# torchmd/mdgrad

Measured on AMD Instinct MI355X. Metric: MD steps/sec (fwd+adjoint), 108-atom LJ NHC, higher is better.
Workload: dtype f32; 1 GPU; FCC 3^3 LJ(1,1) 108 atoms rc 2.5 NHC(Q50,5) dt 0.005, 49 steps+RDF loss+adjoint, 16384 rep/GPU; replicas_per_gpu=16384, md_steps_per_pass=802816, parallelism=replica-dp1, rdf_fused_into_trajectory_kernels=True

## Files before the change

mdgrad_amd/csrc/traj_ring.hpp:

```cpp

__device__ __forceinline__ float ring_move(float v, int src4) {
    return __builtin_bit_cast(float, __builtin_amdgcn_ds_bpermute(src4, __builtin_bit_cast(int, v)));
}
__device__ __forceinline__ f32x2 ring_move(f32x2 v, int src4) { return f32x2{ring_move(v.x, src4), ring_move(v.y, src4)}; }
__device__ __forceinline__ float row_up(float v) {
    return __builtin_bit_cast(float, __builtin_amdgcn_update_dpp(0, __builtin_bit_cast(int, v), 0x101, 0xf, 0xf, true));
}
__device__ __forceinline__ float row_down(float v) {
    return __builtin_bit_cast(float, __builtin_amdgcn_update_dpp(0, __builtin_bit_cast(int, v), 0x111, 0xf, 0xf, true));
}
__device__ __forceinline__ float lane0(float v) {
    return __builtin_bit_cast(float, __builtin_amdgcn_readfirstlane(__builtin_bit_cast(int, v)));
}
__device__ __forceinline__ f32x2 rcp2(f32x2 v) { return f32x2{__builtin_amdgcn_rcpf(v.x), __builtin_amdgcn_rcpf(v.y)}; }
__device__ __forceinline__ float hsum(f32x2 v) { return v.x + v.y; }

__device__ __forceinline__ f32x2 min_image_diag2_near_fused(f32x2 d, float invf, float h) {
    const float M = 12582912.f;
    const f32x2 o = __builtin_elementwise_fma(d, f32x2{invf, invf}, f32x2{M, M}) - M;
    return d - o * h;
}

struct Vec3x2 { f32x2 x, y, z; };
__device__ __forceinline__ Vec3x2 vzero() { const f32x2 z = {0.f, 0.f}; return Vec3x2{z, z, z}; }
__device__ __forceinline__ Vec3x2 ring_move(const Vec3x2& a, int s) { return Vec3x2{ring_move(a.x, s), ring_move(a.y, s), ring_move(a.z, s)}; }

struct RingLJ {
    float sig2, rc2, m1a, m1b, ka, kb, tsa, tsb, tea, teb;
    float a6, a12, b6, b12, sg6, sg12;
    float ivx, ivy, ivz, hx, hy, hz;
    float fvx, fvy, fvz;
    TermConst t0;
    uint32_t rcm;
    bool full;
};

__device__ __forceinline__ RingLJ ring_constants(const TrajArgs& A, int m = 0) {
    const TermConst t0 = term_prepare(A.terms.t[m], A.theta);
    const float e4 = 4.f * t0.k1, cq = t0.c;
    RingLJ K;
    K.sig2 = t0.k0 * t0.k0; K.rc2 = t0.rc2;
    K.m1a = 6.f * e4 * cq; K.m1b = 12.f * e4;
    K.ka = (42.f + 6.f) * e4 * cq; K.kb = (156.f + 12.f) * e4;
    K.tsa = 18.f * e4 * t0.k2 * cq; K.tsb = 72.f * e4 * t0.k2;
    K.tea = 12.f * cq; K.teb = 24.f;
    K.sg6 = K.sig2 * K.sig2 * K.sig2; K.sg12 = K.sg6 * K.sg6;
    K.a6 = K.m1a * K.sg6; K.a12 = K.m1b * K.sg12; K.b6 = K.ka * K.sg6; K.b12 = K.kb * K.sg12;
    K.ivx = A.cell.inv[0]; K.ivy = A.cell.inv[4]; K.ivz = A.cell.inv[8];
    K.hx = A.cell.h[0]; K.hy = A.cell.h[4]; K.hz = A.cell.h[8];
    K.t0 = t0;
    K.rcm = t0.rc2 > 0.f ? __float_as_uint(t0.rc2) - 1u : 0u;
    K.fvx = A.inv_f[0]; K.fvy = A.inv_f[1]; K.fvz = A.inv_f[2];
    K.full = A.lean && A.fused_image && !(A.prm.n_atoms & 1);
    return K;
}

struct RingRdf {
    uint32_t* hist; float inv_h, tlo, fmax;
    const float4* tab; float ulo, inv_hu, tmax;
    float toff, tzero;
    const float2* ttab; unsigned long long* tg64; int32_t* tflag; float tgw, tu0, tinv_du, ttmax, tlim; int tgmax;
};

__device__ __forceinline__ void ring_table_scatter2(const RingRdf& X, int idx, float va, float vb) {
    if (!(fmaxf(fabsf(va), fabsf(vb)) < X.tlim)) *X.tflag = 4;
    atomicAdd(X.tg64 + idx, fx64(va));
    atomicAdd(X.tg64 + idx + 1, fx64(vb));
}

constexpr bool ring_level_force(int level) { return level == 1 || level == 2; }

template <int LEVEL, int IMAGE, bool CROSS, bool JSIDE, int RDF, int KIND, bool SUMS = true>
__device__ __forceinline__ void ring_pair(const RingLJ& K, const RingRdf& X, const Vec3x2& qi, const Vec3x2& wi,
                                          const Vec3x2& qj, const Vec3x2& wj, bool v0, bool v1, bool r0, bool r1,
                                          Vec3x2& fi, Vec3x2& gi, Vec3x2& fj, Vec3x2& gj, f32x2 (&TH)[MDG_MAX_THETA],
                                          Vec3x2& ri, Vec3x2& rj) {
    f32x2 dx = (CROSS ? qj.x.yx : qj.x) - qi.x, dy = (CROSS ? qj.y.yx : qj.y) - qi.y,
          dz = (CROSS ? qj.z.yx : qj.z) - qi.z;
// ... 165 lines not shown
    const bool vi0 = 2 * lane < N, vi1 = 2 * lane + 1 < N;
    f32x2* sqx = lds; f32x2* sqy = lds + 64; f32x2* sqz = lds + 128;
    f32x2* swx = lds + 192; f32x2* swy = lds + 256; f32x2* swz = lds + 320;
    ring_lds_fence();
    sqx[lane] = q.x; sqy[lane] = q.y; sqz[lane] = q.z;
    if constexpr (LEVEL >= 2) { swx[lane] = w.x; swy[lane] = w.y; swz[lane] = w.z; }
    ring_lds_fence();
    Vec3x2 fi = vzero(), gi = vzero(), fj = vzero(), gj = vzero(), ri = vzero(), rj = vzero();
    f32x2 S[MDG_MAX_THETA], D[MDG_MAX_THETA];
#pragma unroll
    for (int k = 0; k < MDG_MAX_THETA; ++k) { S[k] = f32x2{0.f, 0.f}; D[k] = S[k]; }
    static_assert(!FULL || !MASK, "the full ring has no selection mask");
    static_assert(!FULL || NEAR, "the full ring runs on the window form of the minimum image");
    constexpr int IMAGE = NEAR ? (FULL ? 2 : 1) : 0;
    const int nsteps = (nl - 1) >> 1;
    if (!FULL || lane < nl) {
    {
        const bool v = FULL || (vi0 && vi1);
        bool vm = v;
        if constexpr (MASK) vm = v && ((ring_mask_word(M.w, lane >> 4) >> (2 * (lane & 15) + 1)) & 1u);
        ring_pair<LEVEL, IMAGE, true, false, RDF, KIND, SUMS>(K, X, q, w, q, w, vm, vm, v, RDF == 2 && v, fi, gi, fj, gj, D, ri, rj);
    }
    const int prev = lane < nl ? ((lane == 0 ? nl : lane) - 1) * 4 : lane * 4;
    int idx = lane;
    Vec3x2 qj, wj = vzero();
#pragma unroll 1
    for (int k = 1; k <= nsteps; ++k) {
        idx -= 1; idx = idx < 0 ? idx + nl : idx;
        qj.x = sqx[idx]; qj.y = sqy[idx]; qj.z = sqz[idx];
        if constexpr (ring_level_force(LEVEL)) fj = ring_move(fj, prev);
        if constexpr (LEVEL >= 2) { wj.x = swx[idx]; wj.y = swy[idx]; wj.z = swz[idx]; gj = ring_move(gj, prev); }
        if constexpr (RDF == 2) rj = ring_move(rj, prev);
        const bool vj0 = FULL || 2 * idx < N, vj1 = FULL || 2 * idx + 1 < N;
        const bool s0 = FULL || (vi0 && vj0), s1 = FULL || (vi1 && vj1), c0 = FULL || (vi0 && vj1), c1 = FULL || (vi1 && vj0);
        bool ms0 = s0, ms1 = s1, mc0 = c0, mc1 = c1;
        if constexpr (MASK) {
            const uint32_t b0 = ring_mask_word(M.w, idx >> 4) >> (2 * (idx & 15)), b1 = ring_mask_word(M.w + 4, idx >> 4) >> (2 * (idx & 15));
            ms0 = s0 && (b0 & 1u); mc0 = c0 && (b0 & 2u); mc1 = c1 && (b1 & 1u); ms1 = s1 && (b1 & 2u);
        }
        ring_pair<LEVEL, IMAGE, false, true, RDF, KIND, SUMS>(K, X, q, w, qj, wj, ms0, ms1, s0, s1, fi, gi, fj, gj, S, ri, rj);
        ring_pair<LEVEL, IMAGE, true, true, RDF, KIND, SUMS>(K, X, q, w, qj, wj, mc0, mc1, c0, c1, fi, gi, fj, gj, S, ri, rj);
    }
    if (!(nl & 1)) {
        idx -= 1; idx = idx < 0 ? idx + nl : idx;
        qj.x = sqx[idx]; qj.y = sqy[idx]; qj.z = sqz[idx];
        if constexpr (LEVEL >= 2) { wj.x = swx[idx]; wj.y = swy[idx]; wj.z = swz[idx]; }
        const bool vj0 = FULL || 2 * idx < N, vj1 = FULL || 2 * idx + 1 < N;
        const bool s0 = FULL || (vi0 && vj0), s1 = FULL || (vi1 && vj1), c0 = FULL || (vi0 && vj1), c1 = FULL || (vi1 && vj0);
        bool ms0 = s0, ms1 = s1, mc0 = c0, mc1 = c1;
        if constexpr (MASK) {
            const uint32_t b0 = ring_mask_word(M.w, idx >> 4) >> (2 * (idx & 15)), b1 = ring_mask_word(M.w + 4, idx >> 4) >> (2 * (idx & 15));
            ms0 = s0 && (b0 & 1u); mc0 = c0 && (b0 & 2u); mc1 = c1 && (b1 & 1u); ms1 = s1 && (b1 & 2u);
        }
        const bool once = RDF == 2 || 2 * lane < nl;
        Vec3x2 fu = vzero(), gu = vzero(), ru = vzero();
        ring_pair<LEVEL, IMAGE, false, false, RDF, KIND, SUMS>(K, X, q, w, qj, wj, ms0, ms1, s0 && once, s1 && once, fi, gi, fu, gu, D, ri, ru);
        ring_pair<LEVEL, IMAGE, true, false, RDF, KIND, SUMS>(K, X, q, w, qj, wj, mc0, mc1, c0 && once, c1 && once, fi, gi, fu, gu, D, ri, ru);
    }
    }
    int home = lane + nsteps; home = home >= nl ? home - nl : home;
    home = (lane < nl ? home : lane) * 4;
    if constexpr (ring_level_force(LEVEL)) {
        fj = ring_move(fj, home);
        f.x = fi.x + fj.x; f.y = fi.y + fj.y; f.z = fi.z + fj.z;
    }
    if constexpr (LEVEL >= 2) {
        gj = ring_move(gj, home);
        g.x = -(gi.x + gj.x); g.y = -(gi.y + gj.y); g.z = -(gi.z + gj.z);
        if constexpr (SUMS) {
#pragma unroll
            for (int k = 0; k < MDG_MAX_THETA; ++k)
                th[k] = 2.f * hsum(S[k]) + hsum(D[k]);
        }
    }
    if constexpr (RDF == 2) {
        rj = ring_move(rj, home);
        rq.x = ri.x + rj.x; rq.y = ri.y + rj.y; rq.z = ri.z + rj.z;
    } else {
        rq = vzero();
    }
}

__device__ __forceinline__ bool ring_near(const RingLJ& K, const Vec3x2& q) {
    const f32x2 sx = q.x * K.ivx, sy = q.y * K.ivy, sz = q.z * K.ivz;
    bool out = false;
    out |= !(sx.x > -0.24f && sx.x < 1.24f) | !(sx.y > -0.24f && sx.y < 1.24f);
    out |= !(sy.x > -0.24f && sy.x < 1.24f) | !(sy.y > -0.24f && sy.y < 1.24f);
    out |= !(sz.x > -0.24f && sz.x < 1.24f) | !(sz.y > -0.24f && sz.y < 1.24f);
    return __builtin_amdgcn_ballot_w64(out) == 0;
}

template <int LEVEL, int RDF, int KIND, bool MASK, bool SUMS = true>
__device__ __forceinline__ void ring_force(const RingLJ& K, const RingRdf& X, const RingMask& M, bool with_rdf, int N, int lane,
                                           const Vec3x2& q, const Vec3x2& w, Vec3x2& f, Vec3x2& g, float (&th)[MDG_MAX_THETA],
                                           Vec3x2& rq, f32x2* __restrict__ lds) {
    const bool near = ring_near(K, q);
    constexpr bool FULL_OK = !MASK && KIND == KIND_LJ126;
    const bool full = FULL_OK && near && K.full;
    if constexpr (RDF != 0) {
        if (with_rdf) {
            if (full) ring_sweep<LEVEL, true, RDF, KIND, MASK, SUMS, FULL_OK>(K, X, M, N, lane, q, w, f, g, th, rq, lds);
            else if (near) ring_sweep<LEVEL, true, RDF, KIND, MASK, SUMS>(K, X, M, N, lane, q, w, f, g, th, rq, lds);
            else ring_sweep<LEVEL, false, RDF, KIND, MASK, SUMS>(K, X, M, N, lane, q, w, f, g, th, rq, lds);
            return;
        }
    }
    if constexpr (LEVEL >= 1) {
        if (full) ring_sweep<LEVEL, true, 0, KIND, MASK, SUMS, FULL_OK>(K, X, M, N, lane, q, w, f, g, th, rq, lds);
        else if (near) ring_sweep<LEVEL, true, 0, KIND, MASK, SUMS>(K, X, M, N, lane, q, w, f, g, th, rq, lds);
        else ring_sweep<LEVEL, false, 0, KIND, MASK, SUMS>(K, X, M, N, lane, q, w, f, g, th, rq, lds);
// ... 346 lines not shown
        gth[0] += nve ? (gs * 0.5f * h) * 2.f : gs * h;
        gth[1] += nve ? (ge * 0.5f * h) * 2.f : ge * h;
    } else {
#pragma unroll
        for (int k = 0; k < kind_ntheta(KIND); ++k) {
            const float tk = wave_sum(th[k]);
            gth[k] += nve ? (tk * 0.5f * h) * 2.f : tk * h;
        }
    }
}

constexpr int RING_TABLE_WAVES = 8;
constexpr int RING_RDF_ADJ_WAVES = 4;
constexpr int ring_adj_waves(bool rdf, int kind) { return kind == KIND_TABLE ? RING_TABLE_WAVES : (rdf ? RING_RDF_ADJ_WAVES : 1); }
constexpr int RING_PARK_VECS = 4;
constexpr bool ring_adj_parks(int kind, bool mask, int nt, bool ft) { return kind == KIND_LJ126 && !mask && nt == 1 && ft; }
constexpr int ring_adj_slab(bool parks) { return (6 + (parks ? 3 * RING_PARK_VECS : 0)) * 64; }
__device__ __forceinline__ void ring_park(f32x2* __restrict__ park, int slot, int lane, const Vec3x2& a) {
    f32x2* p = park + slot * 192 + lane;
    p[0] = a.x; p[64] = a.y; p[128] = a.z;
}
__device__ __forceinline__ Vec3x2 ring_unpark(const f32x2* __restrict__ park, int slot, int lane) {
    const f32x2* p = park + slot * 192 + lane;
    return Vec3x2{p[0], p[64], p[128]};
}

template <bool NHC, bool RDF, int KIND, bool MASK, int NT, bool FT>
__device__ __forceinline__ void ring_adj_intervals(const TrajArgs& A, const RingRdfArgs& F, const RingLJ (&K)[NT], RingRdf& X,
                                                   const RingMask (&M)[NT], bool live, size_t fr, int lane, f32x2* __restrict__ lds,
                                                   Vec3x2& lv, Vec3x2& lq, float& lp, float (&gth)[NT][MDG_MAX_THETA]) {
    constexpr bool PARK = ring_adj_parks(KIND, MASK, NT, FT);
    static_assert(NT == 1 || !RDF, "several terms: no fused observable");
    const int N = A.prm.n_atoms, T = A.prm.n_frames, C = A.prm.n_chains, N3 = 3 * N;
    f32x2* park = lds + 6 * 64;
    f32x2 ms = {1.f, 1.f};
    if (2 * lane < N) ms.x = A.mass[2 * lane];
    if (2 * lane + 1 < N) ms.y = A.mass[2 * lane + 1];
    const f32x2 ims = rcp2(ms);
    const float Qk = ring_chain_mass(A, lane);
    const float iQ0 = 1.f / A.prm.Q[0];
    for (int i = T - 1; i >= 1; --i) {
        const float h = A.t[i] - A.t[i - 1];
        Vec3x2 q = ring_load(A.q_t + (fr + i) * N3, N, lane);
        float pv = (NHC && lane < C) ? A.pv_t[(fr + i) * C + lane] : 0.f;
        Vec3x2 w, f, dq, rq = vzero(), ru;
        float th[NT][MDG_MAX_THETA];
        if constexpr (NHC) { w.x = lv.x * ims; w.y = lv.y * ims; w.z = lv.z * ims; } else w = lv;
        const bool with_rdf = RDF && ring_frame_selected(F, i);
        if constexpr (KIND == KIND_TABLE) X.tgw = (NHC || !live) ? 0.f : 0.5f * h * A.terms.t[0].c;
        if constexpr (PARK) {
            if constexpr (NHC) ring_park(park, 0, lane, lv);
            ring_park(park, 1, lane, lq);
        }
        ring_force_terms<FT ? 3 : 2, RDF ? 2 : 0, KIND, MASK, NT, !NHC>(K, X, M, with_rdf, N, lane, q, w, f, dq, th, rq, lds);
        if constexpr (PARK) {
            if constexpr (NHC) lv = ring_unpark(park, 0, lane); else lv = w;
            lq = ring_unpark(park, 1, lane);
        }
        if constexpr (FT) f = ring_load(A.f_t + (fr + i) * N3, N, lane);
        Vec3x2 v = ring_load(A.v_t + (fr + i) * N3, N, lane);
        if (with_rdf) { lq.x += rq.x; lq.y += rq.y; lq.z += rq.z; }
        Vec3x2 lvh, lqh;
        if constexpr (NHC) {
            const Vec3x2 p{v.x * ms, v.y * ms, v.z * ms};
            const float ke = 0.5f * wave_sum(ring_dot(p, v)), slv = wave_sum(ring_dot(lv, v));
            const float pv0 = lane0(pv), lp0 = lane0(lp), c0 = pv0 * iQ0;
            const float pb = ring_bath_rhs(A, lane, Qk, pv, ke), gp = ring_bath_vjp(A, lane, Qk, pv, lp, slv);
            const float hh = 0.5f * h;
#define MDG_RING_HALF(c)                                                                     \
            {                                                                                \
                const f32x2 a = (f.c - c0 * p.c) * ims;                                      \
                const f32x2 Gv = -c0 * lv.c + lq.c + 2.f * ms * v.c * lp0;                   \
                const f32x2 vhalf = 0.5f * (-a) * h;                     \
                q.c = q.c + (v.c + vhalf) * h;                           \
                v.c = v.c + vhalf;                                                           \
                lvh.c = lv.c + Gv * hh;                                            \
                lqh.c = lq.c + dq.c * hh;                                          \
            }
            MDG_RING_HALF(x) MDG_RING_HALF(y) MDG_RING_HALF(z)
#undef MDG_RING_HALF
            const float lph = lp + gp * hh;
            pv = pv + 0.5f * (-pb) * h;
            w.x = lvh.x * ims; w.y = lvh.y * ims; w.z = lvh.z * ims;
            if constexpr (KIND == KIND_TABLE) X.tgw = live ? 0.5f * h * A.terms.t[0].c : 0.f;
            if constexpr (PARK) {
                ring_park(park, 0, lane, lv); ring_park(park, 1, lane, lq);
                ring_park(park, 2, lane, lvh); ring_park(park, 3, lane, lqh);
            }
            ring_force_terms<2, 0, KIND, MASK, NT>(K, X, M, false, N, lane, q, w, f, dq, th, ru, lds);
            if constexpr (PARK) {
                lv = ring_unpark(park, 0, lane); lq = ring_unpark(park, 1, lane);
                lvh = ring_unpark(park, 2, lane); lqh = ring_unpark(park, 3, lane);
            }
            const float slm = wave_sum(ring_dot(lvh, v));
            const float cm = lane0(pv) * iQ0, lpm0 = lane0(lph);
            const float gpm = ring_bath_vjp(A, lane, Qk, pv, lph, slm);
            const Vec3x2 gv = A.g_v ? ring_load(A.g_v + (fr + i - 1) * N3, N, lane) : vzero();
            const Vec3x2 gq = A.g_q ? ring_load(A.g_q + (fr + i - 1) * N3, N, lane) : vzero();
#define MDG_RING_FULL(c)                                                                     \
            {                                                                                \
                const f32x2 Gv = -cm * lvh.c + lqh.c + 2.f * ms * v.c * lpm0;                \
                lv.c = (lv.c + Gv * h) + gv.c;                               \
                lq.c = (lq.c + dq.c * h) + gq.c;                                   \
            }
            MDG_RING_FULL(x) MDG_RING_FULL(y) MDG_RING_FULL(z)
#undef MDG_RING_FULL
            float nlp = lp + gpm * h;
// ... 40 lines not shown
    constexpr int NWV = ring_adj_waves(RDF, KIND);
    const int wid = NWV > 1 ? __builtin_amdgcn_readfirstlane((int)(threadIdx.x >> 6)) : 0, lane = threadIdx.x & 63, N3 = 3 * N;
    const bool live = NWV == 1 || (int)(blockIdx.x * NWV + wid) < A.prm.n_rep;
    const int rep = NWV == 1 ? (int)blockIdx.x : (live ? (int)(blockIdx.x * NWV + wid) : A.prm.n_rep - 1);
    RingLJ K[NT];
    RingMask M[NT];
#pragma unroll
    for (int m = 0; m < NT; ++m) {
        K[m] = ring_constants(A, m);
        M[m] = RingMask{};
        if constexpr (MASK) M[m] = ring_mask_load(A.terms.t[m].mask, N, lane);
    }
    RingRdf X{};
    int ntab = 0;
    if constexpr (RDF) {
        float hu;
        int ncell;
        rdf_u_grid(F.mu, F.nbins, F.reach_bins, X.ulo, hu, ncell);
        float4* tab = reinterpret_cast<float4*>(smr);
        for (int n = threadIdx.x; n < ncell; n += blockDim.x) tab[n] = F.tab[n];
        if (threadIdx.x == 0) tab[ncell] = make_float4(0.f, 0.f, 0.f, 0.f);
        X.tab = tab; X.inv_hu = 1.0f / hu; X.toff = -X.ulo * X.inv_hu; X.tzero = (float)ncell;
        X.tmax = fminf((float)ncell, (F.rc * F.rc - X.ulo) * X.inv_hu);
        ntab = ncell + 1;
        __syncthreads();
    }
    f32x2* lds = reinterpret_cast<f32x2*>(smr + 4 * ntab) + wid * ring_adj_slab(ring_adj_parks(KIND, MASK, NT, FT));
    if constexpr (KIND == KIND_TABLE) {
        const MdgPairTerm& t0 = A.terms.t[0];
        float2* ttab = reinterpret_cast<float2*>(smr + 4 * ntab + NWV * 6 * 64 * 2);
        unsigned long long* tg = reinterpret_cast<unsigned long long*>(ttab + t0.p);
        int32_t* tflag = reinterpret_cast<int32_t*>(tg + 2 * t0.p);
        const float* thp = A.theta + t0.theta_off;
        for (int g = threadIdx.x; g < t0.p; g += blockDim.x) ttab[g] = make_float2(thp[2 * g], thp[2 * g + 1]);
        for (int g = threadIdx.x; g < 2 * t0.p; g += blockDim.x) tg[g] = 0ull;
        if (threadIdx.x == 0) *tflag = 0;
        X.ttab = ttab; X.tg64 = tg; X.tflag = tflag; X.tgw = 0.f;
        X.tlim = fx64_limit((double)NWV * (double)(T > 1 ? T - 1 : 1) * (double)N * (double)N);
        X.tu0 = t0.a; X.tinv_du = 1.f / t0.phi; X.ttmax = (float)(t0.p - 1); X.tgmax = t0.p - 2;
        __syncthreads();
    }
    const size_t fr = (size_t)rep * T;
    Vec3x2 lv = A.g_v ? ring_load(A.g_v + (fr + T - 1) * N3, N, lane) : vzero();
    Vec3x2 lq = A.g_q ? ring_load(A.g_q + (fr + T - 1) * N3, N, lane) : vzero();
    float lp = (nhc && lane < C && A.g_pv) ? A.g_pv[(fr + T - 1) * C + lane] : 0.f;
    float gth[NT][MDG_MAX_THETA];
#pragma unroll
    for (int m = 0; m < NT; ++m)
#pragma unroll
        for (int k = 0; k < MDG_MAX_THETA; ++k) gth[m][k] = 0.f;
    if (nhc) ring_adj_intervals<true, RDF, KIND, MASK, NT, FT>(A, F, K, X, M, live, fr, lane, lds, lv, lq, lp, gth);
    else ring_adj_intervals<false, RDF, KIND, MASK, NT, FT>(A, F, K, X, M, live, fr, lane, lds, lv, lq, lp, gth);
    if constexpr (RDF) {
        if (ring_frame_selected(F, 0)) {
            const Vec3x2 q = ring_load(A.q_t + fr * N3, N, lane), wu = vzero();
            Vec3x2 fu, gu, rq = vzero();
            float tu[MDG_MAX_THETA];
            ring_force<0, 2, KIND, MASK>(K[0], X, M[0], true, N, lane, q, wu, fu, gu, tu, rq, lds);
            lq.x += rq.x; lq.y += rq.y; lq.z += rq.z;
        }
    }
    if (live) {
        ring_store(A.adj_v0 + (size_t)rep * N3, lv, N, lane);
        ring_store(A.adj_q0 + (size_t)rep * N3, lq, N, lane);
        if (nhc && lane < C && A.adj_pv0) A.adj_pv0[(size_t)rep * C + lane] = lp;
    }
    if constexpr (KIND == KIND_TABLE) {
        __syncthreads();
        if (A.adj_theta) {
            const int M2 = 2 * A.terms.t[0].p, KT = A.terms.n_theta_total;
            const bool worst = (*X.tflag & 4) != 0;
            const double inv = 1.0 / (double)A.terms.t[0].c;
            float* out = A.adj_theta + (size_t)(blockIdx.x * NWV) * KT + A.terms.t[0].theta_off;
            for (int g = threadIdx.x; g < M2; g += blockDim.x)
                out[g] = worst ? __builtin_inff() : (float)((double)(long long)X.tg64[g] * inv);
            if (wid > 0 && live) {
                float* mine = A.adj_theta + (size_t)rep * KT + A.terms.t[0].theta_off;
                for (int g = lane; g < M2; g += 64) mine[g] = 0.f;
            }
        }
        return;
    }
    if (live && lane == 0 && A.adj_theta) {
#pragma unroll
        for (int m = 0; m < NT; ++m) {
            float* out = A.adj_theta + (size_t)rep * A.terms.n_theta_total + A.terms.t[m].theta_off;
#pragma unroll
            for (int k = 0; k < MDG_MAX_THETA; ++k)
                if (k < A.terms.t[m].n_theta) out[k] = gth[m][k];
        }
    }
}
```

mdgrad_amd/csrc/traj_small.hip:

```cpp
#include "common.hpp"
#include <cmath>

namespace {

struct TrajArgs {
    MdgTrajParams prm;
    MdgCell cell;
    MdgTerms terms;
    const float* theta;
    const float* mass;
    const float* t;
    const float* v0; const float* q0; const float* pv0;
    float* v_t; float* q_t; float* pv_t;
    const float* g_v; const float* g_q; const float* g_pv;
    float* adj_v0; float* adj_q0; float* adj_pv0; float* adj_theta;
    int32_t* nonfinite;
    int ld;
    uint16_t* code;
    int freq;
    long long count0;
    float* f_t;
    int lean;
    float inv_f[3];
    int fused_image;
};

constexpr int KMAX_ALL = MDG_MAX_TERMS * MDG_MAX_THETA;
constexpr int RED_FLOATS = 16 * (KMAX_ALL + 2);
#define KMAX (NT * MDG_MAX_THETA)

template <int LEVEL, int LDC, bool EVEN, bool NEAR>
__device__ __forceinline__ void force_lj126_packed(const TrajArgs& A, int tpa_log2, const float* __restrict__ q,
                                                   const float* __restrict__ w, float* __restrict__ f,
                                                   float* __restrict__ dq, float& th_sig, float& th_eps, bool th_on) {
    const int N = A.prm.n_atoms, LD = LDC ? LDC : A.ld;
    const int TPA = 1 << tpa_log2;
    const int slots = blockDim.x >> tpa_log2;
    const int slot = threadIdx.x >> tpa_log2, sub = threadIdx.x & (TPA - 1);
    const TermConst t0 = term_prepare(A.terms.t[0], A.theta);
    const float sig2 = t0.k0 * t0.k0, e4 = 4.f * t0.k1, cq = t0.c, rc2 = t0.rc2;
    const float m1a = 6.f * e4 * cq, m1b = 12.f * e4;
    const float ka = (42.f + 6.f) * e4 * cq, kb = (156.f + 12.f) * e4;
    const float tsa = 18.f * e4 * t0.k2 * cq, tsb = 72.f * e4 * t0.k2;
    const float tea = 12.f * cq, teb = 24.f;
    const float ivx = A.cell.inv[0], ivy = A.cell.inv[4], ivz = A.cell.inv[8];
    const float hx = A.cell.h[0], hy = A.cell.h[4], hz = A.cell.h[8];
    f32x2 S6 = {0.f, 0.f}, S12 = {0.f, 0.f};
    for (int i = slot; i < N; i += slots) {
        const float xi = q[i], yi = q[LD + i], zi = q[2 * LD + i];
        float wxi = 0.f, wyi = 0.f, wzi = 0.f;
        if (LEVEL >= 2) { wxi = w[i]; wyi = w[LD + i]; wzi = w[2 * LD + i]; }
        f32x2 fx = {0.f, 0.f}, fy = fx, fz = fx, gx = fx, gy = fx, gz = fx;
#pragma unroll 2
        for (int j = 2 * sub; j < N; j += 2 * TPA) {
            const bool live2 = EVEN || j + 1 < N;
            const float* qj = q + j;
            const f32x2 qx = *reinterpret_cast<const f32x2*>(qj), qy = *reinterpret_cast<const f32x2*>(qj + LD),
                        qz = *reinterpret_cast<const f32x2*>(qj + 2 * LD);
            f32x2 dx = qx - xi, dy = qy - yi, dz = qz - zi;
            f32x2 ax = {0.f, 0.f}, ay = ax, az = ax;
            if (LEVEL >= 2) {
                const float* wj = w + j;
                ax = wxi - *reinterpret_cast<const f32x2*>(wj); ay = wyi - *reinterpret_cast<const f32x2*>(wj + LD);
                az = wzi - *reinterpret_cast<const f32x2*>(wj + 2 * LD);
            }
            if constexpr (NEAR) {
                dx = min_image_diag2_near(dx, ivx, hx); dy = min_image_diag2_near(dy, ivy, hy);
                dz = min_image_diag2_near(dz, ivz, hz);
            } else {
                dx = min_image_diag2(dx, ivx, hx); dy = min_image_diag2(dy, ivy, hy); dz = min_image_diag2(dz, ivz, hz);
            }
            const f32x2 d2 = norm2_ref2(dx, dy, dz);
            const bool ok0 = (d2.x != 0.f) && (d2.x < rc2);
            const bool ok1 = live2 && (d2.y != 0.f) && (d2.y < rc2);
            const f32x2 i2 = {ok0 ? __builtin_amdgcn_rcpf(d2.x) : 0.f, ok1 ? __builtin_amdgcn_rcpf(d2.y) : 0.f};
            const f32x2 s2 = sig2 * i2;
            const f32x2 s6 = s2 * s2 * s2;
// ... 671 lines not shown
        }
        return;
    }
    if (tid == 0 && A.adj_theta) {
        const int KT = A.terms.n_theta_total;
#pragma unroll
        for (int m = 0; m < NT; ++m)
#pragma unroll
            for (int k = 0; k < MDG_MAX_THETA; ++k)
                if (m < A.terms.n_terms && k < A.terms.t[m].n_theta)
                    A.adj_theta[(size_t)rep * KT + A.terms.t[m].theta_off + k] = gth[m * MDG_MAX_THETA + k];
    }
}

#include "traj_ring.hpp"

constexpr int RING_TABLE_MAX_NODES = 2048;
size_t ring_table_adj_lds(int nodes);
size_t device_lds_per_block() {
    static size_t cached = 0;
    if (!cached) {
        int dev = 0, v = 0;
        if (hipGetDevice(&dev) != hipSuccess || hipDeviceGetAttribute(&v, hipDeviceAttributeMaxSharedMemoryPerBlock, dev) != hipSuccess || v <= 0)
            v = 64 * 1024;
        cached = (size_t)v;
    }
    return cached;
}

int ring_kind(const MdgPairTerm& t);
bool ring_form(const MdgTrajParams& p, const MdgCell& cell, const MdgTerms& terms) {
    const MdgPairTerm& t = terms.t[0];
    if (t.kind == MDG_PAIR_TABLE) {
        const char* e = getenv("MDG_RING_TABLE");
        return !(e && e[0] == '0') && terms.n_terms == 1 && cell.diag && !t.mask && t.p <= RING_TABLE_MAX_NODES && p.n_atoms <= 128 &&
               ring_table_adj_lds(t.p) <= device_lds_per_block();
    }
    if (terms.n_terms == 2 || terms.n_terms == 3) {
        bool any_mask = false;
        for (int m = 0; m < terms.n_terms; ++m) {
            const MdgPairTerm& u = terms.t[m];
            if (u.kind != MDG_PAIR_LJ || ring_kind(u) != ring_kind(t)) return false;
            any_mask = any_mask || u.mask != nullptr;
        }
        return cell.diag && p.n_atoms <= 128 && any_mask;
    }
    return terms.n_terms == 1 && cell.diag && (!t.mask || t.kind == MDG_PAIR_LJ) && t.kind >= 0 && t.kind <= MDG_PAIR_YUKAWA &&
           p.n_atoms <= 128;
}
int ring_lean() {
    static const int lean = [] { const char* e = getenv("MDG_RING_LEAN"); return !(e && e[0] == '0') ? 1 : 0; }();
    return lean;
}
bool fused_image_multiplier(float h, float inv, float* out) {
    if (!(h > 0.f) || !(inv > 0.f) || !std::isfinite(h) || !std::isfinite(inv)) return false;
    auto rounded = [inv](float d) { volatile float s = d * inv; return (float)s; };
    float tau = 0.5f * h;
    if (!(tau > 0.f) || !std::isfinite(rounded(2.f * h))) return false;
    int budget = 64;
    while (rounded(std::nextafterf(tau, 0.f)) > 0.5f && --budget > 0) tau = std::nextafterf(tau, 0.f);
    while (!(rounded(tau) > 0.5f) && --budget > 0) tau = std::nextafterf(tau, INFINITY);
    if (budget <= 0) return false;
    const double below = (double)std::nextafterf(tau, 0.f), at = (double)tau;
    for (int k = 0; k <= 8; ++k) {
        float c = inv;
        const int steps = (k + 1) / 2;
        for (int s = 0; s < steps; ++s) c = std::nextafterf(c, (k & 1) ? 0.f : INFINITY);
        if (below * (double)c <= 0.5 && 0.5 < at * (double)c) { *out = c; return true; }
    }
    return false;
}
void set_fused_image(TrajArgs& a) {
    a.fused_image = a.cell.diag ? 1 : 0;
    for (int k = 0; k < 3; ++k) {
        a.inv_f[k] = a.cell.inv[4 * k];
        if (a.fused_image && !fused_image_multiplier(a.cell.h[4 * k], a.cell.inv[4 * k], &a.inv_f[k])) a.fused_image = 0;
    }
}
bool use_ring(const MdgTrajParams& p, const MdgCell& cell, const MdgTerms& terms) {
    return ring_form(p, cell, terms) && (p.block == 64 || (p.block == 0 && p.n_rep >= 1024));
}
int ring_kind(const MdgPairTerm& t) {
    if (t.kind == MDG_PAIR_TABLE) return KIND_TABLE;
    return (t.kind == MDG_PAIR_LJ && t.p == 12 && (t.q == 6 || t.c == 0.f)) ? KIND_LJ126 : t.kind;
}
size_t ring_table_lds(const MdgTerms& terms, bool adjoint) {
    if (terms.t[0].kind != MDG_PAIR_TABLE) return 0;
    return sizeof(float) * (size_t)(adjoint ? 6 : 2) * terms.t[0].p + 16;
}
#define MDG_RING_FT , true
#define MDG_RING_LAUNCH(KERNEL, RDF_, TAIL, grid, block, lds, st, ...)                                        \
    do {                                                                                                      \
        const bool masked_ = terms->t[0].mask != nullptr;                                                     \
        const int nt_ = terms->n_terms;               \
        switch (ring_kind(terms->t[0])) {                                                                     \
        case KIND_LJ126:                                                                                      \
            if (nt_ == 2) hipLaunchKernelGGL((KERNEL<false, KIND_LJ126, true, 2 TAIL>), grid, block, lds, st, __VA_ARGS__);    \
            else if (nt_ == 3) hipLaunchKernelGGL((KERNEL<false, KIND_LJ126, true, 3 TAIL>), grid, block, lds, st, __VA_ARGS__); \
            else if (masked_) hipLaunchKernelGGL((KERNEL<RDF_, KIND_LJ126, true, 1 TAIL>), grid, block, lds, st, __VA_ARGS__);    \
            else hipLaunchKernelGGL((KERNEL<RDF_, KIND_LJ126, false, 1 TAIL>), grid, block, lds, st, __VA_ARGS__);               \
            break;                                                                                            \
        case MDG_PAIR_LJ:                                                                                     \
            if (nt_ == 2) hipLaunchKernelGGL((KERNEL<false, MDG_PAIR_LJ, true, 2 TAIL>), grid, block, lds, st, __VA_ARGS__);   \
            else if (nt_ == 3) hipLaunchKernelGGL((KERNEL<false, MDG_PAIR_LJ, true, 3 TAIL>), grid, block, lds, st, __VA_ARGS__);  \
            else if (masked_) hipLaunchKernelGGL((KERNEL<RDF_, MDG_PAIR_LJ, true, 1 TAIL>), grid, block, lds, st, __VA_ARGS__);   \
            else hipLaunchKernelGGL((KERNEL<RDF_, MDG_PAIR_LJ, false, 1 TAIL>), grid, block, lds, st, __VA_ARGS__);              \
// ... 162 lines not shown
    const char* who = small_who(false, o);
    const bool stale = o.extra == SmallOpt::STALE, rdf = o.extra == SmallOpt::RDF;
    MDG_CHECK_ARG(mass && t_grid && v0 && q0 && v_t && q_t && (!rdf || ((theta || terms->n_theta_total == 0) && o.raw)),
                  "%s: null buffer", who);
    MDG_CHECK_ARG(prm->ensemble == 1 || (pv0 && pv_t), "%s: NHC needs pv0/pv_t", who);
    RdfFinePlan P;
    if ((rc = validate_small_opt(who, prm, cell, terms, o, &P)) != MDG_OK) return rc;
    TrajArgs a{};
    a.prm = *prm; a.cell = *cell; a.terms = *terms; a.theta = theta; a.mass = mass; a.t = t_grid;
    a.v0 = v0; a.q0 = q0; a.pv0 = pv0; a.v_t = v_t; a.q_t = q_t; a.pv_t = pv_t; a.nonfinite = nonfinite;
    hipStream_t st = (hipStream_t)stream;
    if (rdf || (!stale && use_ring(*prm, *cell, *terms))) {
        MDG_CHECK_ARG(theta || terms->n_theta_total == 0, "%s: null theta", who);
        a.f_t = o.f_t; a.lean = ring_lean(); set_fused_image(a);
        if (!rdf) {
            MDG_RING_LAUNCH(traj_fwd_ring_kernel, false, , dim3(prm->n_rep), dim3(64), RING_LDS_FWD + ring_table_lds(*terms, false),
                            st, a, RingRdfArgs{});
            MDG_CHECK_LAUNCH("traj_fwd_ring_kernel");
            return MDG_OK;
        }
        uint32_t* ghist = nullptr;
        MDG_HIP(hipMallocAsync((void**)&ghist, sizeof(uint32_t) * (size_t)P.nfine, st));
        MDG_HIP(hipMemsetAsync(ghist, 0, sizeof(uint32_t) * (size_t)P.nfine, st));
        RingRdfArgs F = ring_rdf_args(*o.rdf, P);
        F.ghist = ghist;
        int grid = (prm->n_rep + RING_RDF_WAVES - 1) / RING_RDF_WAVES;
        if (grid > 256) grid = 256;
        const size_t lds = sizeof(float) * (size_t)((P.nfine + 1) & ~1LL) + RING_RDF_WAVES * RING_LDS_FWD;
        MDG_RING_LAUNCH(traj_fwd_ring_kernel, true, , dim3(grid), dim3(64 * RING_RDF_WAVES), lds, st, a, F);
        rc = mdg_rdf_fine_finish(ghist, P, o.rdf->mu, o.rdf->nbins, o.raw, st);
        (void)hipFreeAsync(ghist, st);
        if (rc) return rc;
        MDG_CHECK_LAUNCH("traj_fwd_ring_kernel<rdf>");
        return MDG_OK;
    }
    SmallGeom g;
    if ((rc = small_geometry(who, prm, terms, theta, false, &g)) != MDG_OK) return rc;
    a.ld = g.ld;
    if (stale) { a.code = o.code; a.freq = o.freq; a.count0 = o.count0; }
    MDG_TRAJ_DISPATCH(traj_fwd_kernel, stale);
    MDG_CHECK_LAUNCH(stale ? "traj_fwd_kernel (stale lists)" : "traj_fwd_kernel");
    return MDG_OK;
}

int traj_adj_small_run(const MdgTrajParams* prm, const MdgCell* cell, const MdgTerms* terms,
                       const float* theta, const float* mass, const float* t_grid,
                       const float* v_t, const float* q_t, const float* pv_t,
                       const float* g_v, const float* g_q, const float* g_pv,
                       float* adj_v0, float* adj_q0, float* adj_pv0, float* adj_theta, void* stream, const SmallOpt& o) {
    int rc = validate(prm, cell, terms);
    if (rc) return rc;
    const char* who = small_who(true, o);
    const bool stale = o.extra == SmallOpt::STALE, rdf = o.extra == SmallOpt::RDF;
    MDG_CHECK_ARG(mass && t_grid && v_t && q_t && adj_v0 && adj_q0 &&
                  (!rdf || ((theta || terms->n_theta_total == 0) && o.g_raw)), "%s: null buffer", who);
    MDG_CHECK_ARG(prm->ensemble == 1 || pv_t, "%s: NHC needs pv_t", who);
    RdfFinePlan P;
    if ((rc = validate_small_opt(who, prm, cell, terms, o, &P)) != MDG_OK) return rc;
    TrajArgs a{};
    a.prm = *prm; a.cell = *cell; a.terms = *terms; a.theta = theta; a.mass = mass; a.t = t_grid;
    a.v_t = const_cast<float*>(v_t); a.q_t = const_cast<float*>(q_t); a.pv_t = const_cast<float*>(pv_t);
    a.g_v = g_v; a.g_q = g_q; a.g_pv = g_pv;
    a.adj_v0 = adj_v0; a.adj_q0 = adj_q0; a.adj_pv0 = adj_pv0; a.adj_theta = adj_theta;
    hipStream_t st = (hipStream_t)stream;
    if (rdf || (!stale && use_ring(*prm, *cell, *terms))) {
        MDG_CHECK_ARG(theta || terms->n_theta_total == 0, "%s: null theta", who);
        a.f_t = o.f_t; a.lean = ring_lean(); set_fused_image(a);
        if (!rdf) {
            const bool rt = terms->t[0].kind == MDG_PAIR_TABLE;
            const int wpw = rt ? RING_TABLE_WAVES : 1;
            const size_t lds = wpw * ring_adj_wave_lds(*terms, o.f_t != nullptr) + ring_table_lds(*terms, true);
            if (o.f_t)
                MDG_RING_LAUNCH(traj_adj_ring_kernel, false, MDG_RING_FT, dim3((prm->n_rep + wpw - 1) / wpw), dim3(64 * wpw), lds,
                                st, a, RingRdfArgs{});
            else
                MDG_RING_LAUNCH(traj_adj_ring_kernel, false, , dim3((prm->n_rep + wpw - 1) / wpw), dim3(64 * wpw), lds,
                                st, a, RingRdfArgs{});
            MDG_CHECK_LAUNCH("traj_adj_ring_kernel");
            return MDG_OK;
        }
        const int wpw = RING_RDF_ADJ_WAVES;
        const size_t lds = sizeof(float4) * (size_t)(P.ncell + 1) + wpw * ring_adj_wave_lds(*terms, o.f_t != nullptr);
        MDG_CHECK_ARG(lds <= device_lds_per_block(), "%s: %zu bytes of LDS per workgroup exceed the device's limit", who, lds);
        float4* tab = nullptr;
        MDG_HIP(hipMallocAsync((void**)&tab, sizeof(float4) * (size_t)P.ncell, st));
        rc = mdg_rdf_bwd_table_u(o.rdf->mu, o.rdf->coeff, o.rdf->nbins, o.g_raw, P, tab, st);
        if (rc == MDG_OK) {
            RingRdfArgs F = ring_rdf_args(*o.rdf, P);
            F.tab = tab;
            const dim3 grid((prm->n_rep + wpw - 1) / wpw), block(64 * wpw);
            if (o.f_t) MDG_RING_LAUNCH(traj_adj_ring_kernel, true, MDG_RING_FT, grid, block, lds, st, a, F);
            else MDG_RING_LAUNCH(traj_adj_ring_kernel, true, , grid, block, lds, st, a, F);
        }
        (void)hipFreeAsync(tab, st);
        if (rc) return rc;
        MDG_CHECK_LAUNCH("traj_adj_ring_kernel<rdf>");
        return MDG_OK;
    }
    SmallGeom g;
    if ((rc = small_geometry(who, prm, terms, theta, true, &g)) != MDG_OK) return rc;
    a.ld = g.ld;
    if (stale) { a.code = o.code; a.freq = o.freq; a.count0 = o.count0; }
    MDG_TRAJ_DISPATCH(traj_adj_kernel, stale);
    MDG_CHECK_LAUNCH(stale ? "traj_adj_kernel (stale lists)" : "traj_adj_kernel");
    return MDG_OK;
}

}

extern "C" int mdg_traj_small_fits(int n_atoms, int table_nodes) {
    return n_atoms > 0 && table_nodes >= 0 && small_lds(n_atoms, table_nodes, false) <= SMALL_LDS_MAX &&
           small_lds(n_atoms, table_nodes, true) <= SMALL_LDS_MAX;
}

extern "C" int mdg_min_image_fused_inv(float h, float inv, float* inv_fused) {
    float c = 0.f;
    const bool ok = inv_fused && fused_image_multiplier(h, inv, &c);
    if (ok) *inv_fused = c;
    return ok ? 1 : 0;
}
// ... 115 lines not shown
```

mdgrad_amd/ops.py:

```python
import ctypes as C
import math
import weakref

import numpy as np
import torch
from array import array as _array

from . import _lib
from . import _torch_ops
from ._lib import MdgPairTerm, MdgTerms, MdgTrajParams, check, ptr, stream_ptr, require_gpu


def build_mask(n_atoms, index_tuple=None, ex_pairs=None, device=None):
    if index_tuple is None and ex_pairs is None:
        return None
    keep = torch.ones(n_atoms, n_atoms, dtype=torch.bool)
    if index_tuple is not None:
        a = torch.as_tensor(list(index_tuple[0]), dtype=torch.long)
        b = torch.as_tensor(list(index_tuple[1]), dtype=torch.long)
        sel = torch.zeros(n_atoms, n_atoms, dtype=torch.bool)
        sel[a[:, None], b[None, :]] = True
        keep &= sel | sel.t()
    if ex_pairs is not None:
        ex = torch.as_tensor(ex_pairs, dtype=torch.long).reshape(-1, 2).cpu()
# ... 1048 lines not shown

    def __init__(self, obs, start, stride):
        import weakref
        self.obs = weakref.ref(obs)
        self.mu = obs.offsets.detach().to(torch.float32).contiguous()
        self.nbins, self.coeff, self.spacing = int(obs.nbins), float(obs.coeff), float(obs.spacing)
        self.mu0 = float(obs.r_axis[0])
        self.cutoff, self.n_atoms = float(obs.cutoff_boundary), int(obs.natoms)
        self.cell = tuple(float(x) for x in obs.cell.tolist())
        self.start, self.stride = int(start), int(stride)

    def struct(self):
        return _lib.MdgRdfFuse(self.mu.data_ptr(), self.nbins, self.coeff, self.mu0, self.spacing, self.cutoff, self.start,
                               self.stride)

    def matches(self, obs, start, stride):
        return self.obs() is obs and self.start == int(start) and self.stride == int(stride)

    def fits(self, spec, dev):
        cs = spec.cell_struct
        return (self.obs() is not None and self.n_atoms == spec.n_atoms and self.mu.device == dev
                and bool(cs.diag) and all(abs(cs.h[4 * c] - self.cell[c]) <= 1e-6 * abs(self.cell[c]) for c in range(3)))


def fused_traj(v0, q0, pv0, t, theta, spec, time_dim=None):
    outs = FusedTrajFn.apply(v0, q0, pv0, t, theta, spec, True)
    n = 3 if spec.ensemble == 0 else 2
    tag_trajectory(outs[1], spec, outs[n] if len(outs) > n else None,
                   (1 if v0.dim() == 3 else 0) if time_dim is None else time_dim)
    return tuple(outs[:n])


def tag_trajectory(q_t, spec, raw, time_dim):
    q_t._mdg_traj = (spec, time_dim, spec.rdf_hint if raw is not None else None, raw)


def _stale_launch(ctx, spec, R, T, dev, calls, launch):
    integ = spec._integrator
    if getattr(integ, "_stale_code", None) is None and ctx.stale_code is not None:
        integ._stale_code = ctx.stale_code
    code = integ.stale_lists(R, spec.n_atoms, dev, large=ctx.large)
    launch(int(ctx.stale_freq), int(integ.update_count), ptr(code))
    integ.update_count += calls * (T - 1)
    integ._stale_fused_dirty = True
    return code


class FusedTrajFn(torch.autograd.Function):

    @staticmethod
    def forward(ctx, v0, q0, pv0, t, theta, spec, fuse=False):
        lib = _lib.load()
        require_gpu(v0, "v0"), require_gpu(q0, "q0"), require_gpu(t, "t")
        batched = v0.dim() == 3
        R = v0.shape[0] if batched else 1
        N, T = spec.n_atoms, t.shape[0]
        dev = v0.device
        nhc = spec.ensemble == 0
        Cn = len(spec.Q)
        v0c, q0c = v0.detach().contiguous(), q0.detach().contiguous()
        pv0c = pv0.detach().contiguous() if nhc else None
        tc = t.detach().to(torch.float32).contiguous()
        thc = theta.detach().contiguous() if theta is not None and theta.numel() else None
        v_t = torch.empty(R, T, N, 3, device=dev)
        q_t = torch.empty(R, T, N, 3, device=dev)
        pv_t = torch.empty(R, T, Cn, device=dev) if nhc else None
        prm = spec.params(R, T)
        ctx.large, ctx.stale_freq, ctx.table = bool(spec.large), int(spec.stale_freq), bool(spec.table)
        ctx.ws, ctx.lists_ok, ctx.stale_code = None, False, None
        fuse = spec.rdf_hint if fuse else None
        if fuse is not None and (spec.large or spec.table or thc is None or not fuse.fits(spec, dev)
                                 or not lib.mdg_traj_rdf_supported(C.byref(prm), C.byref(spec.cell_struct),
                                                                   C.byref(spec.terms), C.byref(fuse.struct()))):
            fuse = None
        ctx.fuse = fuse
        raw = None
        f_t = None
        if not ctx.large and not ctx.stale_freq and lib.mdg_traj_ring_taken(
                C.byref(prm), C.byref(spec.cell_struct), C.byref(spec.terms)):
            f_t = torch.empty(R, T, N, 3, device=dev)
        ctx.f_t = f_t
        args = (C.byref(prm), C.byref(spec.cell_struct), C.byref(spec.terms), ptr(thc), ptr(spec.mass), ptr(tc),
                ptr(v0c), ptr(q0c), ptr(pv0c), ptr(v_t), ptr(q_t), ptr(pv_t))

        def run(fn, *extras):
            check(fn(*args, *extras, stream_ptr(dev)), fn.__name__)

        if ctx.large:
            ws = torch.empty(int(lib.mdg_traj_large_workspace(R, N, T, spec.n_theta_total)), device=dev)
            flags = torch.zeros(8, dtype=torch.int32, device=dev)
            out = (ptr(ws), ptr(flags))
        else:
            bad = torch.zeros(R, dtype=torch.int32, device=dev)
            out = (ptr(bad),)
        if fuse is not None:
            raw = torch.empty(fuse.nbins, device=dev)
            run(lib.mdg_traj_fwd_small_rdf_ft, ptr(f_t), *out, C.byref(fuse.struct()), ptr(raw))
        elif ctx.stale_freq:
            fn = lib.mdg_traj_fwd_large_stale if ctx.large else lib.mdg_traj_fwd_small_stale
            ctx.stale_code = _stale_launch(ctx, spec, R, T, dev, 2, lambda *tail: run(fn, *out, *tail))
        elif ctx.large:
            run(lib.mdg_traj_fwd_large, *out)
        else:
            run(lib.mdg_traj_fwd_small_ft, ptr(f_t), *out)
        if ctx.large:
            fl = flags.tolist()
# ... 13 lines not shown
                    "mdgrad_amd: a pair came closer than table_rmin * cutoff = %.4g, below the first node of the "
                    "tabulated pair potential; lower `table_rmin` on the integrator or set `fused_table = False` "
                    "to evaluate the module per pair" % math.sqrt(spec.u0))
        ctx.spec, ctx.batched, ctx.nhc = spec, batched, nhc
        ctx.nonfinite = bad
        saved = [tc, v_t, q_t] + ([pv_t] if nhc else []) + ([thc] if thc is not None else [])
        ctx.has_theta = thc is not None
        ctx.save_for_backward(*saved)
        outs = (v_t, q_t, pv_t) if nhc else (v_t, q_t)
        if not batched:
            outs = tuple(o[0] for o in outs)
        if raw is not None:
            outs = outs + (raw,)
        return outs

    @staticmethod
    def backward(ctx, *grads):
        lib = _lib.load()
        spec, nhc = ctx.spec, ctx.nhc
        saved = list(ctx.saved_tensors)
        tc, v_t, q_t = saved[0], saved[1], saved[2]
        pv_t = saved[3] if nhc else None
        thc = saved[-1] if ctx.has_theta else None
        R, T, N = v_t.shape[0], v_t.shape[1], spec.n_atoms
        dev = v_t.device
        if ctx.nonfinite is not None and bool((ctx.nonfinite & 1).any()):
            raise RuntimeError("mdgrad_amd: the forward trajectory reached a non-finite state (time step too large "
                               "or overlapping atoms); its adjoint is undefined")

        def prep(g, like):
            if g is None:
                return None
            g = g.detach()
            if not ctx.batched:
                g = g[None]
            return g.expand_as(like).contiguous()

        gv = prep(grads[0], v_t)
        gq = prep(grads[1], q_t)
        gp = prep(grads[2], pv_t) if nhc else None
        fuse = ctx.fuse
        g_raw = grads[3 if nhc else 2] if fuse is not None else None
        if g_raw is not None and ctx.needs_input_grad[3]:
            sel = q_t[:, fuse.start::fuse.stride].contiguous()
            gsel = torch.empty_like(sel)
            cs = spec.cell_struct
            check(lib.mdg_rdf_bwd_uniform(ptr(sel), sel.shape[0] * sel.shape[1], N, C.byref(cs), fuse.cutoff, None,
                                          ptr(fuse.mu), fuse.spacing, fuse.coeff, fuse.nbins,
                                          ptr(g_raw.detach().to(torch.float32).contiguous()), ptr(gsel), stream_ptr(dev)),
                  "mdg_rdf_bwd")
            gq = torch.zeros_like(q_t) if gq is None else gq.clone()
            gq[:, fuse.start::fuse.stride] += gsel
            g_raw = None
        adj_v = torch.empty(R, N, 3, device=dev)
        adj_q = torch.empty(R, N, 3, device=dev)
        adj_p = torch.empty(R, len(spec.Q), device=dev) if nhc else None
        KT = spec.n_theta_total
        adj_th = torch.zeros(R, KT, device=dev) if KT else None
        prm = spec.params(R, T)
        table, ws, lists_ok = ctx.table, ctx.ws, ctx.lists_ok
        frames = (ptr(thc), ptr(spec.mass), ptr(tc), ptr(v_t), ptr(q_t), ptr(pv_t))
        grads_ = (ptr(gv), ptr(gq), ptr(gp), ptr(adj_v), ptr(adj_q), ptr(adj_p), ptr(adj_th))

        def run(fn, terms, *extras, prm=prm, f_t=()):
            check(fn(C.byref(prm), C.byref(spec.cell_struct), C.byref(terms), *frames, *f_t, *grads_, *extras,
                     stream_ptr(dev)), fn.__name__)

        def launch(terms, search=False):
            if g_raw is not None:
                gr = g_raw.detach().to(torch.float32).contiguous()
                run(lib.mdg_traj_adj_small_rdf_ft, terms, C.byref(fuse.struct()), ptr(gr), f_t=(ptr(ctx.f_t),))
                return None
            if ctx.stale_freq:
                flags = torch.zeros(8, dtype=torch.int32, device=dev) if ctx.large else None
                fn = lib.mdg_traj_adj_large_stale if ctx.large else lib.mdg_traj_adj_small_stale
                out = (ptr(ws), ptr(flags)) if ctx.large else ()
                _stale_launch(ctx, spec, R, T, dev, 3, lambda *tail: run(fn, terms, *out, *tail))
                return flags
            if ctx.large:
                pl = type(prm).from_buffer_copy(prm)
                for search in ((search,) if (search or not lists_ok or spec.block == -1) else (False, True)):
                    pl.block = -1 if (search or not lists_ok or spec.block == -1) else 0
                    flags = torch.zeros(8, dtype=torch.int32, device=dev)
                    run(lib.mdg_traj_adj_large, terms, ptr(ws), ptr(flags), prm=pl)
                    if pl.block == -1 or not int(flags[5]):
                        break
                    LARGE_STATS["adjoint_redone_with_searches"] += 1
                return flags
            run(lib.mdg_traj_adj_small_ft, terms, f_t=(ptr(ctx.f_t),))
            return None

        def check_large(flags):
            f = flags.tolist()
            if f[0]:
                raise RuntimeError("mdgrad_amd: an atom has %d neighbours within the cutoff in the adjoint sweep; "
                                   "the fused large-N kernel holds 256 per atom" % f[0])
            if f[1]:
                raise RuntimeError("mdgrad_amd: non-finite state in the fused large-N adjoint sweep")
            return f

        if table:
            lam = max([float(g.abs().max()) for g in (gv, gq) if g is not None] + [1e-30])
            h = float((tc[1:] - tc[:-1]).abs().max())
            est = max(0.5 * h * 2.0 * spec.terms.t[0].cutoff * lam / float(spec.mass.min()), 1e-30)
            S = max(-100, min(100, int(math.floor(30 - math.log2(est)))))
            for attempt in range(4):
                terms = type(spec.terms).from_buffer_copy(spec.terms)
                terms.t[0].c = 2.0 ** S
                flags = launch(terms)
                bad = bool(check_large(flags)[2]) if flags is not None else not bool(torch.isfinite(adj_th[:, 0]).all())
                if not bad:
                    break
                S -= 14
            else:
                raise RuntimeError("mdgrad_amd: the table-gradient accumulation overflowed (adjoint magnitudes "
                                   "above ~2^%d of the incoming gradients)" % (40 - S))
        else:
            flags = launch(spec.terms)
            if flags is not None:
                check_large(flags)
        if not ctx.batched:
            adj_v, adj_q = adj_v[0], adj_q[0]
            adj_p = adj_p[0] if nhc else None
        gth = adj_th.sum(0) if adj_th is not None else None
        g_t = None
        if ctx.needs_input_grad[3]:
            g_t = _time_vjps(spec, tc, v_t, q_t, pv_t, gv, gq, gp)
        return adj_v, adj_q, adj_p, g_t, gth, None, None


def _time_vjps(spec, t, v_t, q_t, pv_t, gv, gq, gp):
    integ = spec._integrator
    if integ is None:
        raise NotImplementedError("mdgrad_amd: dL/dt needs the integrator behind the fused spec")
    R, T = v_t.shape[0], v_t.shape[1]
    nhc = pv_t is not None
    stacked = spec.n_rep > 1
    zero = lambda like: torch.zeros_like(like)
    out = torch.zeros(T, device=v_t.device, dtype=t.dtype)
    with torch.no_grad():
        for k in range(1, T):
            frames = [None] if stacked else range(R)
            for r in frames:
                if stacked:
                    v, q = v_t[:, k].reshape(-1, 3), q_t[:, k].reshape(-1, 3)
                    pv = pv_t[:, k] if nhc else None
                    g_v = gv[:, k].reshape(-1, 3) if gv is not None else zero(v)
                    g_q = gq[:, k].reshape(-1, 3) if gq is not None else zero(q)
                    g_p = (gp[:, k] if gp is not None else zero(pv)) if nhc else None
                else:
                    v, q = v_t[r, k], q_t[r, k]
                    pv = pv_t[r, k] if nhc else None
                    g_v = gv[r, k] if gv is not None else zero(v)
                    g_q = gq[r, k] if gq is not None else zero(q)
                    g_p = (gp[r, k] if gp is not None else zero(pv)) if nhc else None
                integ.model._reset_topology(q)
                F = integ.model.force(q)
                if nhc:
                    a, _, b = integ.rhs_from_force((v, q, pv), F)
                    out[k] += (a * g_v).sum() + (v * g_q).sum() + (b * g_p).sum()
                else:
                    out[k] += (F * g_v).sum() + (v * g_q).sum()
        out[0] = -out[1:].sum()
    return out


RDF_LIST_ATOMS = 2048


def _rdf_pair_table(g_raw, mu, coeff, cutoff, nodes=4096):
    lo = max(float(mu[0]) - 6.0 / math.sqrt(-2.0 * coeff), 0.05)
    u0, u1 = lo * lo, float(cutoff) ** 2
    du = (u1 - u0) / (nodes - 1)
    r = (u0 + du * torch.arange(nodes, device=mu.device, dtype=torch.float32)).sqrt()[:, None]
# ... 1182 lines not shown
```

Measured before the change: 41.82 million MD steps/s.

## Halve unmasked ring tail pairs and skip unread adjoint outputs

In the unmasked ring, the even-length tail step now splits the self/cross pair work across lanes by swapping qj components and scattering reactions back to the mate lane. Previously each lane evaluated both pairs with half masked off. The adjoint also skips gradient-term work in the first cold step when no incoming v gradient exists, and skips the frame-0 RDF pass and the adj_v0/adj_q0 stores when those outputs aren't requested. The skipping is gated by an environment flag that is on by default. It adds cross-lane permutes and relies on the zero-gradient assumptions being correct.

Result: faster. 43.83 million MD steps/s, median of 6 (+4.8%).

```diff
diff --git a/mdgrad_amd/csrc/traj_ring.hpp b/mdgrad_amd/csrc/traj_ring.hpp
--- a/mdgrad_amd/csrc/traj_ring.hpp
+++ b/mdgrad_amd/csrc/traj_ring.hpp
@@ -24,6 +24,8 @@
 struct Vec3x2 { f32x2 x, y, z; };
 __device__ __forceinline__ Vec3x2 vzero() { const f32x2 z = {0.f, 0.f}; return Vec3x2{z, z, z}; }
 __device__ __forceinline__ Vec3x2 ring_move(const Vec3x2& a, int s) { return Vec3x2{ring_move(a.x, s), ring_move(a.y, s), ring_move(a.z, s)}; }
+__device__ __forceinline__ f32x2 ring_swap_if(bool c, f32x2 v) { return f32x2{c ? v.y : v.x, c ? v.x : v.y}; }
+__device__ __forceinline__ Vec3x2 ring_swap_if(bool c, const Vec3x2& a) { return Vec3x2{ring_swap_if(c, a.x), ring_swap_if(c, a.y), ring_swap_if(c, a.z)}; }
 
 struct RingLJ {
     float sig2, rc2, m1a, m1b, ka, kb, tsa, tsb, tea, teb;
@@ -295,10 +297,32 @@
             const uint32_t b0 = ring_mask_word(M.w, idx >> 4) >> (2 * (idx & 15)), b1 = ring_mask_word(M.w + 4, idx >> 4) >> (2 * (idx & 15));
             ms0 = s0 && (b0 & 1u); mc0 = c0 && (b0 & 2u); mc1 = c1 && (b1 & 1u); ms1 = s1 && (b1 & 2u);
         }
-        const bool once = RDF == 2 || 2 * lane < nl;
-        Vec3x2 fu = vzero(), gu = vzero(), ru = vzero();
-        ring_pair<LEVEL, IMAGE, false, false, RDF, KIND, SUMS>(K, X, q, w, qj, wj, ms0, ms1, s0 && once, s1 && once, fi, gi, fu, gu, D, ri, ru);
-        ring_pair<LEVEL, IMAGE, true, false, RDF, KIND, SUMS>(K, X, q, w, qj, wj, mc0, mc1, c0 && once, c1 && once, fi, gi, fu, gu, D, ri, ru);
+        if constexpr (MASK) {
+            const bool once = RDF == 2 || 2 * lane < nl;
+            Vec3x2 fu = vzero(), gu = vzero(), ru = vzero();
+            ring_pair<LEVEL, IMAGE, false, false, RDF, KIND, SUMS>(K, X, q, w, qj, wj, ms0, ms1, s0 && once, s1 && once, fi, gi, fu, gu, D, ri, ru);
+            ring_pair<LEVEL, IMAGE, true, false, RDF, KIND, SUMS>(K, X, q, w, qj, wj, mc0, mc1, c0 && once, c1 && once, fi, gi, fu, gu, D, ri, ru);
+        } else {
+            const bool up = 2 * lane >= nl;
+            qj.x = ring_swap_if(up, qj.x); qj.y = ring_swap_if(up, qj.y); qj.z = ring_swap_if(up, qj.z);
+            if constexpr (LEVEL >= 2) { wj.x = ring_swap_if(up, wj.x); wj.y = ring_swap_if(up, wj.y); wj.z = ring_swap_if(up, wj.z); }
+            const bool a0 = FULL || (up ? c0 : s0), a1 = FULL || (up ? c1 : s1);
+            const int mate = (FULL || lane < nl) ? idx * 4 : lane * 4;
+            Vec3x2 fa = vzero(), ga = vzero(), ra = vzero();
+            ring_pair<LEVEL, IMAGE, false, true, RDF, KIND, SUMS>(K, X, q, w, qj, wj, a0, a1, a0, a1, fi, gi, fa, ga, S, ri, ra);
+            if constexpr (ring_level_force(LEVEL)) {
+                fa = ring_move(ring_swap_if(up, fa), mate);
+                fi.x += fa.x; fi.y += fa.y; fi.z += fa.z;
+            }
+            if constexpr (LEVEL >= 2) {
+                ga = ring_move(ring_swap_if(up, ga), mate);
+                gi.x += ga.x; gi.y += ga.y; gi.z += ga.z;
+            }
+            if constexpr (RDF == 2) {
+                ra = ring_move(ring_swap_if(up, ra), mate);
+                ri.x += ra.x; ri.y += ra.y; ri.z += ra.z;
+            }
+        }
     }
     }
     int home = lane + nsteps; home = home >= nl ? home - nl : home;
@@ -751,7 +775,19 @@
             if constexpr (NHC) ring_park(park, 0, lane, lv);
             ring_park(park, 1, lane, lq);
         }
-        ring_force_terms<FT ? 3 : 2, RDF ? 2 : 0, KIND, MASK, NT, !NHC>(K, X, M, with_rdf, N, lane, q, w, f, dq, th, rq, lds);
+        constexpr bool COLD_OK = FT && NT == 1 && KIND != KIND_TABLE;
+        const bool cold = COLD_OK && A.skip_unread && !A.g_v && i == T - 1;
+        if (cold) {
+            if constexpr (COLD_OK) {
+                ring_force<0, RDF ? 2 : 0, KIND, MASK>(K[0], X, M[0], with_rdf, N, lane, q, w, f, dq, th[0], rq, lds);
+                const f32x2 nz = {-0.f, -0.f};
+                dq = Vec3x2{nz, nz, nz};
+#pragma unroll
+                for (int k = 0; k < MDG_MAX_THETA; ++k) th[0][k] = 0.f;
+            }
+        } else {
+            ring_force_terms<FT ? 3 : 2, RDF ? 2 : 0, KIND, MASK, NT, !NHC>(K, X, M, with_rdf, N, lane, q, w, f, dq, th, rq, lds);
+        }
         if constexpr (PARK) {
             if constexpr (NHC) lv = ring_unpark(park, 0, lane); else lv = w;
             lq = ring_unpark(park, 1, lane);
@@ -898,7 +934,7 @@
     if (nhc) ring_adj_intervals<true, RDF, KIND, MASK, NT, FT>(A, F, K, X, M, live, fr, lane, lds, lv, lq, lp, gth);
     else ring_adj_intervals<false, RDF, KIND, MASK, NT, FT>(A, F, K, X, M, live, fr, lane, lds, lv, lq, lp, gth);
     if constexpr (RDF) {
-        if (ring_frame_selected(F, 0)) {
+        if (ring_frame_selected(F, 0) && (A.adj_q0 || !A.skip_unread)) {
             const Vec3x2 q = ring_load(A.q_t + fr * N3, N, lane), wu = vzero();
             Vec3x2 fu, gu, rq = vzero();
             float tu[MDG_MAX_THETA];
@@ -907,8 +943,8 @@
         }
     }
     if (live) {
-        ring_store(A.adj_v0 + (size_t)rep * N3, lv, N, lane);
-        ring_store(A.adj_q0 + (size_t)rep * N3, lq, N, lane);
+        if (A.adj_v0) ring_store(A.adj_v0 + (size_t)rep * N3, lv, N, lane);
+        if (A.adj_q0) ring_store(A.adj_q0 + (size_t)rep * N3, lq, N, lane);
         if (nhc && lane < C && A.adj_pv0) A.adj_pv0[(size_t)rep * C + lane] = lp;
     }
     if constexpr (KIND == KIND_TABLE) {
diff --git a/mdgrad_amd/csrc/traj_small.hip b/mdgrad_amd/csrc/traj_small.hip
--- a/mdgrad_amd/csrc/traj_small.hip
+++ b/mdgrad_amd/csrc/traj_small.hip
@@ -23,6 +23,7 @@
     int lean;
     float inv_f[3];
     int fused_image;
+    int skip_unread;
 };
 
 constexpr int KMAX_ALL = MDG_MAX_TERMS * MDG_MAX_THETA;
@@ -800,6 +801,10 @@
     static const int lean = [] { const char* e = getenv("MDG_RING_LEAN"); return !(e && e[0] == '0') ? 1 : 0; }();
     return lean;
 }
+int ring_skip_unread() {
+    static const int skip = [] { const char* e = getenv("MDG_RING_SKIP_UNREAD"); return !(e && e[0] == '0') ? 1 : 0; }();
+    return skip;
+}
 bool fused_image_multiplier(float h, float inv, float* out) {
     if (!(h > 0.f) || !(inv > 0.f) || !std::isfinite(h) || !std::isfinite(inv)) return false;
     auto rounded = [inv](float d) { volatile float s = d * inv; return (float)s; };
@@ -1068,7 +1073,8 @@
     if (rc) return rc;
     const char* who = small_who(true, o);
     const bool stale = o.extra == SmallOpt::STALE, rdf = o.extra == SmallOpt::RDF;
-    MDG_CHECK_ARG(mass && t_grid && v_t && q_t && adj_v0 && adj_q0 &&
+    const bool ring = rdf || (!stale && use_ring(*prm, *cell, *terms));
+    MDG_CHECK_ARG(mass && t_grid && v_t && q_t && (ring || (adj_v0 && adj_q0)) &&
                   (!rdf || ((theta || terms->n_theta_total == 0) && o.g_raw)), "%s: null buffer", who);
     MDG_CHECK_ARG(prm->ensemble == 1 || pv_t, "%s: NHC needs pv_t", who);
     RdfFinePlan P;
@@ -1079,9 +1085,9 @@
     a.g_v = g_v; a.g_q = g_q; a.g_pv = g_pv;
     a.adj_v0 = adj_v0; a.adj_q0 = adj_q0; a.adj_pv0 = adj_pv0; a.adj_theta = adj_theta;
     hipStream_t st = (hipStream_t)stream;
-    if (rdf || (!stale && use_ring(*prm, *cell, *terms))) {
+    if (ring) {
         MDG_CHECK_ARG(theta || terms->n_theta_total == 0, "%s: null theta", who);
-        a.f_t = o.f_t; a.lean = ring_lean(); set_fused_image(a);
+        a.f_t = o.f_t; a.lean = ring_lean(); a.skip_unread = ring_skip_unread(); set_fused_image(a);
         if (!rdf) {
             const bool rt = terms->t[0].kind == MDG_PAIR_TABLE;
             const int wpw = rt ? RING_TABLE_WAVES : 1;
diff --git a/mdgrad_amd/ops.py b/mdgrad_amd/ops.py
--- a/mdgrad_amd/ops.py
+++ b/mdgrad_amd/ops.py
@@ -1124,6 +1124,7 @@
     def forward(ctx, v0, q0, pv0, t, theta, spec, fuse=False):
         lib = _lib.load()
         require_gpu(v0, "v0"), require_gpu(q0, "q0"), require_gpu(t, "t")
+        ctx.set_materialize_grads(False)
         batched = v0.dim() == 3
         R = v0.shape[0] if batched else 1
         N, T = spec.n_atoms, t.shape[0]
@@ -1243,9 +1244,10 @@
             gq = torch.zeros_like(q_t) if gq is None else gq.clone()
             gq[:, fuse.start::fuse.stride] += gsel
             g_raw = None
-        adj_v = torch.empty(R, N, 3, device=dev)
-        adj_q = torch.empty(R, N, 3, device=dev)
-        adj_p = torch.empty(R, len(spec.Q), device=dev) if nhc else None
+        want_state = any(ctx.needs_input_grad[0:3]) or ctx.f_t is None
+        adj_v = torch.empty(R, N, 3, device=dev) if want_state else None
+        adj_q = torch.empty(R, N, 3, device=dev) if want_state else None
+        adj_p = torch.empty(R, len(spec.Q), device=dev) if nhc and want_state else None
         KT = spec.n_theta_total
         adj_th = torch.zeros(R, KT, device=dev) if KT else None
         prm = spec.params(R, T)
@@ -1310,7 +1312,7 @@
             flags = launch(spec.terms)
             if flags is not None:
                 check_large(flags)
-        if not ctx.batched:
+        if not ctx.batched and want_state:
             adj_v, adj_q = adj_v[0], adj_q[0]
             adj_p = adj_p[0] if nhc else None
         gth = adj_th.sum(0) if adj_th is not None else None
```
